# Vasilispapg/CVML-GoalNet

Measured on AMD Instinct MI355X. Metric: training clips/sec at batch 64, 16-frame 224² clips; logit MAE vs CPU ref, higher is better.
Workload: dtype f32; 1 GPU; AVM train step (forward + broadcast-MSE + backward + fused Adam), 64 clips x 16 frames = 1024 frames of 3x224x224 + 30x30 MFCC per GPU; dropout live (device masks), BatchNorm train mode; frames_per_gpu=1024, h=224, w=224, parallelism=dp1, ddp_semantics=local BN + local MSE per rank, gradient mean (standard DDP), params=1286754369

## Files before the change

cvml_goalnet_amd/_lib.py:

```python
from __future__ import annotations

import ctypes
import os
from ctypes import c_char_p, c_double, c_float, c_int, c_int64, c_size_t, c_uint32, c_uint64, c_void_p

_HERE = os.path.dirname(os.path.abspath(__file__))
LIB_PATH = os.environ.get("GOALNET_LIB_PATH") or os.path.join(_HERE, "libgoalnet_hip.so")
ABI_VERSION = 7
STAT_PARTS = 1024
ADAM_RANGES_MAX = 32

P = c_void_p


class RowCopy(ctypes.Structure):
    _fields_ = [("src", c_void_p), ("dst", c_void_p), ("row_bytes", c_int64), ("nrows", c_int), ("gather", c_int), ("cursor", c_void_p),
                ("cursor_bias", c_int64)]


class AdamRange(ctypes.Structure):
    _fields_ = [("begin", c_int64), ("count", c_int64), ("skipped", c_int64)]


PROTOTYPES = {
# ... 63 lines not shown
    "goalnet_linear_bwd_dx_split": (c_int, [c_int, P, P, P, c_int64, c_int, c_int64, c_int, P, P]),
    "goalnet_linear_bwd_dw_split": (c_int, [c_int, P, P, P, c_int, c_int64, c_int, P, P]),
    "goalnet_linear_bwd_dx_bf16": (c_int, [P, c_int64, P, P, c_int64, P, c_int64, c_int, c_int64, c_int, c_int, P]),
    "goalnet_linear_bwd_dx_bf16_o16_ok": (c_int, [c_int, c_int64, c_int]),
    "goalnet_linear_bwd_dx_bf16_o16": (c_int, [P, c_int64, P, P, c_int64, c_int, c_int64, c_int, c_int, P]),
    "goalnet_conv3x3_fwd_bf16p_o16_ok": (c_int, [c_int, c_int, c_int, c_int, c_int]),
    "goalnet_conv3x3_fwd_bf16p_o16": (c_int, [P, P, P, c_int, P, c_int, c_int, c_int, c_int, c_int, c_int, P]),
    "goalnet_linear_bwd_dw_bf16": (c_int, [P, c_int64, P, c_int64, P, c_int, c_int64, c_int, c_int, P]),
    "goalnet_linear_fwd_ws_bytes": (c_size_t, [c_int, c_int64, c_int]),
    "goalnet_linear_fwd": (c_int, [P, c_int64, P, P, c_int, P, P, c_int, P, c_int64, P, c_int64, P, c_int64,
                                   c_int, c_int64, c_int, P, c_size_t, P]),
    "goalnet_linear_bwd_dx": (c_int, [P, c_int64, P, P, c_int64, P, c_int64, c_int, c_int64, c_int, P]),
    "goalnet_linear_bwd_dw": (c_int, [P, c_int64, P, c_int64, P, P, c_int, P, P, c_int, c_int64, c_int, P]),
    "goalnet_linear_bwd_dw_adam": (c_int, [P, c_int64, P, c_int64, P, P, c_int, P, P, P, P, c_int, c_int64, c_int,
                                           c_double, c_double, c_double, c_double, P, c_int64, c_float, P]),
    "goalnet_colsum": (c_int, [P, c_int64, c_int, c_int, P, P]),
    "goalnet_mul": (c_int, [P, c_int64, P, c_int64, P, c_int64, c_int, c_int, P]),
    "goalnet_conv1d_fwd": (c_int, [P, P, P, c_int, P, c_int, c_int, c_int, c_int, c_int, c_int, P]),
    "goalnet_conv1d_bwd_ws_bytes": (c_size_t, [c_int, c_int, c_int]),
    "goalnet_conv1d_bwd": (c_int, [P, P, P, P, P, P, c_int, c_int, c_int, c_int, c_int, c_int, P, c_size_t, P]),
    "goalnet_conv1d_bwd_small": (c_int, [P, P, P, P, P, P, P, c_int, c_int, c_int, c_int, c_int, c_int, P]),
    "goalnet_relu_bwd": (c_int, [P, P, P, c_int64, P]),
    "goalnet_mlp_blocks": (c_int, []),
    "goalnet_mlp_fwd": (c_int, [P, c_int64, c_int, P, P, P, P, P, P, P, P, P, P, P, c_int, P, P]),
    "goalnet_mlp_bwd_ws_bytes": (c_size_t, [c_int]),
    "goalnet_mlp_bwd": (c_int, [P, P, P, c_int64, P, c_int64, P, P, P, P, c_int64, P, c_int, c_int, c_int, P, c_size_t, P, P]),
    "goalnet_head_fwd": (c_int, [P, c_int64, P, P, P, P, c_int, c_int, P]),
    "goalnet_head_bwd": (c_int, [P, P, P, c_int64, P, P, c_int64, P, c_int64, P, P, c_int, c_int, P]),
    "goalnet_mse_bcast": (c_int, [P, P, c_int, P, P, P]),
    "goalnet_cubic_resample": (c_int, [P, P, P, c_int64, c_int, c_int, P]),
# ... 75 lines not shown
```

cvml_goalnet_amd/avm.py:

```python
from __future__ import annotations

import math
import os
from typing import List, Optional

import torch
import torch.nn as nn
from torch.nn.parameter import UninitializedParameter

from . import ops
from ._lib import GoalnetError
from .synth import BASE_SEED, DROP_P, TID_DROP

F32 = torch.float32
BN_EPS = 1e-5
BN_MOMENTUM = 0.1
_ALIGN = 64


class _LazyFlags:

    def requires_grad_(self, requires_grad: bool = True):
        for p in self.parameters():
            p.requires_grad = requires_grad
# ... 56 lines not shown
            torch.cuda.current_stream().wait_event(ev)

    def join(self):
        if self.enabled and self.forked:
            torch.cuda.current_stream().wait_stream(self.side)
            self.forked = False
        self.keep.clear()


class _Bwd:

    def __init__(self, model, train, fork):
        self.model, self.train, self.fork = model, train, fork
        self.scratch = {}
        self.dbias = {}
        self.T = train.__contains__

    def any_T(self, *layers):
        return any(f"{layer}.{leaf}" in self.train for layer in layers for leaf in ("weight", "bias"))

    def G(self, name):
        m = self.model
        if name in self.train:
            return m._gflat(name)
        s = m.spec(name)
        if s.kind in ("ohwi", "lin5") and name != "visbl.conv1.weight":
            raise GoalnetError(f"a backward that does not train {name} asked for its gradient")
        t = self.scratch.get(name)
        if t is None:
            t = self.scratch[name] = torch.empty(s.numel, dtype=F32, device=m._device)
# ... 34 lines not shown
    if env == "0":
        return frozenset()
    return frozenset(ch for ch in env.lower() if ch in "a")


def epi_fuse_dw_adam(n, *, plain, synced, precision, train_w5, shadowed, inspected, forced, pieces):
    if forced is False or "a" not in pieces:
        return False
    if inspected and forced is not True:
        return False
    if not (plain and not synced and precision == "fp32" and train_w5 and not shadowed):
        return False
    if n <= EPI_FUSE_SKINNY_ROWS:
        return False
    return forced is True or n >= EPI_FUSE_MIN_ROWS


class AVM(_LazyFlags, nn.Module):
    def __init__(self, audio_included, device=None, seed: Optional[int] = None, precision: str = "fp32", head: str = "regression",
                 num_classes: int = 5):
        super().__init__()
        self.audio_included = audio_included
        if head not in ("regression", "classifier"):
            raise ValueError("head must be 'regression' (the reference's live code) or 'classifier' (its commented-out variant)")
        if not 2 <= num_classes <= 8:
            raise ValueError("num_classes must be in 2..8")
        self.head = head
        self.num_classes = num_classes if head == "classifier" else 1
        if precision not in ("fp32", "bf16", "fp16", "bf16x6", "fp16x3"):
            raise ValueError("precision must be 'fp32' (the reference's arithmetic), 'bf16x6' / 'fp16x3' (fp32 operands as bf16 triples / scaled "
# ... 44 lines not shown
        self.grad_sync = None
        self.stat_sync = None
        self.grad_bf16 = os.environ.get("GOALNET_DZ16", "1") != "0"
        self.act_bf16 = os.environ.get("GOALNET_P16", "1") != "0"
        env = os.environ.get
        self.x6_off = env("GOALNET_X6_OFF") == "1"
        self.x6_linear5 = env("GOALNET_X6_LINEAR5", "1") != "0"
        self.x3_wgrad2 = env("GOALNET_X3_WGRAD2", "1") != "0"
        self.x3_dgrad2 = env("GOALNET_X3_DGRAD2", "1") != "0"
        self.mlp_fused = env("GOALNET_MLP_FUSED", "1") != "0"
        self.small_bn = env("GOALNET_SMALL_BN", "1") != "0"
        self.force_bf5 = env("GOALNET_FORCE_BF5") == "1"
        self.overlap_pair = env("GOALNET_OVERLAP_PAIR", "1") != "0"
        self.epi_fuse = None
        self.epi_fused_dw = 0
        self.keep_ctx = False
        self.last_ctx = None
        self.last_used_w5b = False
        self._side_stream = None
        self.overlap_rows = int(os.environ.get("GOALNET_OVERLAP_ROWS", "64"))
        _ol = os.environ.get("GOALNET_OVERLAP_LARGE")
        self.overlap_large = _ol == "1"
        self.overlap_auto = _ol is None
        self.time_labels = None
        self.kernel_events = None

    @property
    def precision(self) -> str:
        return self._precision

# ... 350 lines not shown
        return self._x6 and ops.linear_split_ok(self._parts, n, k5, 512) and not self.x6_off and self.x6_linear5

    def _mlp_fused(self, n):
        return n <= 16 and self.head == "regression" and self.mlp_fused

    def _bf5(self, n):
        return self._half and (n > 16 or self.force_bf5)

    def _pair(self, n):
        return self._large_overlap(n) and self.overlap_pair

    def _small_bn(self, a, b, n, hc, wc, c):
        return (a.dtype == F32 and b.dtype == F32 and self.stat_sync is None and c <= 512 and n * hc * wc * c <= ops.SMALL_BN_ELEMS
                and self.small_bn)

    def _bn_block(self, y, n, hc, wc, c, i, save, p16=False):
        dev = self._device
        assert p16 or y.dtype == F32
        p = torch.empty(n, hc - 2, wc - 2, c, dtype=self._h16 if p16 else F32, device=dev)
        idx = torch.empty(n, hc - 2, wc - 2, c, dtype=torch.uint8, device=dev) if save else None
        bn = getattr(self.visbl, f"bnorm{i}")
        st = torch.empty(4, c, dtype=F32, device=dev)
        count = n * (hc - 2) * (wc - 2)
        if not self.training:
            ops.pool_bn_eval_fwd(y, p, idx, self._pflat(f"visbl.bnorm{i}.weight"), self._pflat(f"visbl.bnorm{i}.bias"),
                                 bn.running_mean, bn.running_var, BN_EPS, st, n, hc, wc, c)
            return p, idx, st
        if self._small_bn(y, p, n, hc, wc, c):
            ops.pool_bn_fwd_small(y, p, idx, self._pflat(f"visbl.bnorm{i}.weight"), self._pflat(f"visbl.bnorm{i}.bias"),
                                  bn.running_mean, bn.running_var, BN_MOMENTUM, BN_EPS, st, n, hc, wc, c)
# ... 145 lines not shown
        elif not fused_mlp:
            logit = torch.empty(n, dtype=F32, device=dev)
            out = torch.empty(n, dtype=F32, device=dev)
            ops.head_fwd(x, P("fusion.12.weight"), P("fusion.12.bias"), logit, out)
        if save:
            ctx.update(p1=p1, idx1=idx1, st1=st1, p2=p2, idx2=idx2, st2=st2, p3=p3, idx3=idx3, st3=st3,
                       a1=a1, a2=a2, hs=hs, ms=ms, logit=logit, out=out, l1=l1, l2=l2)
        self.last_logit = logit
        self.last_features = cat
        return out, ctx

    def _block_bwd(self, bwd, dbn, ctx, i, n, hc, wc, c):
        dev, G, bias = self._device, bwd.G, bwd.T(f"visbl.conv{i}.bias")
        p, idx, st = ctx[f"p{i}"], ctx[f"idx{i}"], ctx[f"st{i}"]
        npix = n * (hc - 2) * (wc - 2)
        small = self._small_bn(dbn, p, n, hc, wc, c) and not (self._half and i > 1)
        frozen = ctx["eval"]
        if small:
            coef3 = torch.empty(3 * c, dtype=F32, device=dev)
            (ops.bn_bwd_reduce_small_eval if frozen else ops.bn_bwd_reduce_small)(
                dbn, p, st[0], st[1], self._pflat(f"visbl.bnorm{i}.weight"), G(f"visbl.bnorm{i}.weight"), G(f"visbl.bnorm{i}.bias"),
                coef3, n, hc, wc, c)
            dy = torch.empty(n, hc, wc, c, dtype=F32, device=dev)
            dparts = torch.empty(ops.stat_parts(8 * n) * c, dtype=torch.float64, device=dev)
            ops.bnpool_bwd(dbn, p, idx, coef3, dy, dparts, n, hc, wc, c)
            if i > 1 and bias:
                bwd.dbias[i] = (dparts, c)
            return dy
        coef3 = torch.empty(3 * c, dtype=F32, device=dev)
        partials = torch.empty(ops.stat_parts(npix // 64) * 2 * c, dtype=torch.float64, device=dev)
        ops.bn_bwd_reduce(dbn, p, st[0], st[1], partials, npix, c)
        if frozen:
            ops.bn_bwd_finalize_eval(partials, self._pflat(f"visbl.bnorm{i}.weight"), st[1], c,
                                     G(f"visbl.bnorm{i}.weight"), G(f"visbl.bnorm{i}.bias"), coef3)
        else:
            ops.bn_bwd_finalize(partials, self._pflat(f"visbl.bnorm{i}.weight"), st[0], st[1], npix, c,
                                G(f"visbl.bnorm{i}.weight"), G(f"visbl.bnorm{i}.bias"), coef3)
        if self.stat_sync is not None and not frozen:
            scratch = torch.empty(2 * c, dtype=F32, device=dev)
            ops.bn_bwd_finalize(self._global_sums(partials, 2 * c), self._pflat(f"visbl.bnorm{i}.weight"), st[0], st[1],
                                npix * self.stat_sync.world, c, scratch[:c], scratch[c:], coef3)
        dparts = torch.empty(ops.stat_parts(8 * n) * c, dtype=torch.float64, device=dev)
        if self._half and i > 1 and self._bwd16_ok(wc):
            dy = self._padbuf(f"dy{i}", n, hc, wc, c)
            ops.bnpool_bwd_bf16p(dbn, p, idx, coef3, None, dy, dparts, n, hc, wc, c)
        elif self._half and i > 1:
# ... 45 lines not shown
            return None
        if flipped:
            fork.wait(wait_ev)
        else:
            ops.conv3x3_weight_flip(P(wname), wt, cout, cin)
        o16 = out16 and ops.conv3x3_fwd_bf16p_o16_ok(n, hc, wc, cout, cin)
        dx = torch.empty(n, hc, wc, cin, dtype=self._h16 if o16 else F32, device=dev)
        if self._half:
            wtb = ops.cast_bf16(wt, torch.empty(wt.shape, dtype=self._h16, device=dev))
            self._timed("conv_dgrad", flops, ops.conv3x3_fwd_bf16p_o16 if o16 else ops.conv3x3_fwd_bf16p,
                        dy, wtb, None, False, dx, n, hc, wc, cout, cin)
        elif split and split_dgrad:
            wts, awt = self._split_w(wt, cin * 9, cout)
            self._timed("conv_dgrad", flops, ops.conv3x3_fwd_split, self._parts,
                        dys, wts, None, False, dx, n, hc, wc, cout, cin, self._osc(ady, awt))
        else:
            self._timed("conv_dgrad", flops, ops.conv3x3_fwd, dy, None, None, wt, None, False, dx, n, hc, wc, cout, cin)
        if pair:
            wgrad()
        return dx

    def backward_device(self, ctx, dout, on_bucket=None, after_linear5=None, inputs=None, params=True, reduce=0, frozen=None,
                        fused_w5=None):
        need_aud, need_vis = inputs if inputs is not None else (False, False)
        need_aud = need_aud and self.audio_included
        train = frozenset()
        if params:
            frozen = self._frozen_names() if frozen is None else frozenset(frozen)
            self._check_freeze(frozen)
            train = frozenset(s.name for s in self._specs) - frozen
# ... 2 lines not shown
                               "backward ran; call backward after each forward (as the reference's loop does)")
        for i in (3, 2):
            xs = f"x{i - 1}s"
            if not self._half and xs in ctx and f"visbl.conv{i}.weight" in train and ctx[xs + "_gen"] != self._padgen[xs]:
                raise RuntimeError(f"precision='{self.precision}': a second training-mode forward overwrote the saved split operands "
                                   "before backward ran; call backward after each forward (as the reference's loop does)")
        if params:
            self._ensure_garena()
            self._bwd_frozen = frozen
        dev = self._device
        n, h, w = ctx["n"], ctx["h"], ctx["w"]
        bwd = _Bwd(self, train, _Fork(self, self._fork_ok(n) and dout.is_cuda))
        fork, T, G, any_T = bwd.fork, bwd.T, bwd.G, bwd.any_T
        (h1, w1), (hp1, wp1), (hp2, wp2), (hp3, wp3) = self._sizes(h, w)
        P = self._pflat
        need_b1 = need_vis or any_T("visbl.bnorm1", "visbl.conv1")
        need_b2 = need_b1 or any_T("visbl.bnorm2", "visbl.conv2")
        need_b3 = need_b2 or any_T("visbl.bnorm3", "visbl.conv3")
        train_w5 = T("visbl.linear5.weight")
        need_audbl = self.audio_included and (need_aud or any_T("audbl.linear3", "audbl.conv2", "audbl.conv1"))
        need_cat = need_audbl or need_b3 or train_w5 or T("visbl.linear5.bias")
        d_audio = torch.empty(n, 30, ctx["bins"], dtype=F32, device=dev) if need_aud else None
        d_visual = None
        hs, ms = ctx["hs"], ctx["ms"]
        pair = fork.enabled and self._pair(n)
        deferred_l5 = []

        def bucket_done(k):
            if on_bucket:
                fork.join()
# ... 89 lines not shown
                else:
                    ops.linear_bwd_dx_bf16(dz5b, ctx["w5b"], dbn3.view(n, k5), mult=None)
            elif "x3s" in ctx:
                dz5s, adz = self._split_mat(dz5, n, 512)
                if train_w5:
                    osc_w = self._osc(adz, ctx["x3s_amax"])
                    fork.run(lambda: ops.linear_bwd_dw_split(self._parts, dz5s, ctx["x3s"], G("visbl.linear5.weight"), n, k5, 512, oscale=osc_w), dz5s, osc_w)
                bucket_done(1)
                if need_b3:
                    ops.linear_bwd_dx_split(self._parts, dz5s, ctx["w5s"], dbn3.view(n, k5), n, k5, 512, oscale=self._osc(adz, ctx["w5s_amax"]))
            else:
                fuse5 = fused_w5 is not None and train_w5
                if train_w5 and not fuse5:
                    fork.run(lambda: ops.linear_bwd_dw(dz5, p3f, G("visbl.linear5.weight"), scale=st3[2], shift=st3[3], bnC=512), dz)
                bucket_done(1)
                if need_b3:
                    ops.linear_bwd_dx(dz5, P("visbl.linear5.weight"), dbn3.view(n, k5), mult=None)
                if fuse5:
                    fused_w5(dz5, p3f, st3[2], st3[3])
            linear5_done()
        else:
            bucket_done(1)

        b2, b3 = (hp1, wp1, 64, 256), (hp2, wp2, 256, 512)
        dbn2 = dbn1 = None
        if dbn3 is not None:
            dbn2 = self._conv_block_bwd(bwd, 3, dbn3, ctx, n, *b3, wt3, flips_early, flips_ev, pair, out16=dz16 and self._bwd16_ok(wp1),
                                        split_dgrad=True, after_block=lambda: [cb(fork) for cb in deferred_l5], dgrad=need_b2)
        del dbn3
        if dbn2 is not None:
            dbn1 = self._conv_block_bwd(bwd, 2, dbn2, ctx, n, *b2, wt2, flips_early, None, pair, out16=False,
# ... 323 lines not shown
```

cvml_goalnet_amd/csrc/gemm_f32.hip:

```cpp
#include <stdlib.h>

#include "adam.h"
#include "gemm_common.h"
#include "skinny.h"

using namespace goalnet;

namespace {

constexpr int BM = 128, BN = 128, BK = 32;
constexpr int LDR = 128;
constexpr int OP_FLOATS = BM * BK;

__device__ __forceinline__ int kc_off(int row, int chunk) { return row * BK + ((chunk ^ ((row >> 1) & 7)) << 2); }

__device__ __forceinline__ float4 f4zero() { return make_float4(0.f, 0.f, 0.f, 0.f); }
__device__ __forceinline__ float4 f4fma(float4 v, float4 s, float4 t) {
    return make_float4(fmaf(v.x, s.x, t.x), fmaf(v.y, s.y, t.y), fmaf(v.z, s.z, t.z), fmaf(v.w, s.w, t.w));
}

typedef unsigned int u32x4 __attribute__((ext_vector_type(4)));
constexpr unsigned OOB = 0xFFFFFF00u;

__device__ __forceinline__ float4 f4sel(bool v, float4 a) { return v ? a : f4zero(); }
// ... 716 lines not shown
                adam1(pp[q].x, acc[fm][0][e], mm[q].x, vv[q].x, s.b2, s.omb1, s.omb2, ae.eps, s.step_size, s.bc2_sqrt, ae.gs);
                adam1(pp[q].y, acc[fm][1][e], mm[q].y, vv[q].y, s.b2, s.omb1, s.omb2, ae.eps, s.step_size, s.bc2_sqrt, ae.gs);
            }
#pragma unroll
            for (int q = 0; q < 4; ++q) {
                if (ok[q]) {
                    *reinterpret_cast<float2*>(ae.p + idx[q]) = pp[q];
                    *reinterpret_cast<float2*>(ae.m + idx[q]) = mm[q];
                    *reinterpret_cast<float2*>(ae.v + idx[q]) = vv[q];
                }
            }
        }
    }
}

template <class AL, class BL, int STAGES, int EPI>
__global__ __launch_bounds__(256, STAGES == 1 ? AL::ONE_STAGE_BLOCKS : 2) void gemm_f32_epi_kernel(typename AL::P ap, typename BL::P bp, AdamEpi ae,
                                                          int rows, int cols, int64_t ld, int tiles_m, int tiles_n, int m_fast, int ktiles) {
    static_assert(EPI == EPIK_ADAM && !AL::KC && !BL::KC, "the Adam epilogue: both operands row-contiguous");
    const int tid = threadIdx.x;
    int tm, tn;
    tile_of_block(tiles_m, tiles_n, m_fast, tm, tn);
    AdamScalars s = adam_scalars(ae.lr, ae.beta1, ae.beta2, *ae.step + ae.step_bias);
    s.step_size = wave_uniform(s.step_size); s.bc2_sqrt = wave_uniform(s.bc2_sqrt);
    s.b2 = wave_uniform(s.b2); s.omb1 = wave_uniform(s.omb1); s.omb2 = wave_uniform(s.omb2);
    const int lane = tid & 63, wave = tid >> 6;
    const int wm = wave >> 1, wn = wave & 1;
    const int r = lane & 31, h = lane >> 5;
    f32x16 acc[2][2];
    gemm_mainloop<AL, BL, STAGES>(ap, bp, tm, tn, 0, ktiles, tid, acc);
    adam_acc(ae, s, rows, cols, ld, acc, tm, tn, wm, wn, r, h);
}

template <class AL, class BL, int EPI>
int launch_gemm_epi(const char* name, const typename AL::P& ap, const typename BL::P& bp, const AdamEpi& ae, int64_t M, int64_t N,
                    int64_t ld, int ktiles, int m_fast, hipStream_t st) {
    const int64_t tiles_m = (M + BM - 1) / BM, tiles_n = (N + BN - 1) / BN;
    GN_REQUIRE(tiles_m * tiles_n < (1ll << 31), GOALNET_E_SHAPE, "%s: too many tiles", name);
    static const int force_stages = getenv("GOALNET_F32_STAGES") ? atoi(getenv("GOALNET_F32_STAGES")) : 0;
    const dim3 grid((unsigned)(tiles_m * tiles_n), 1, 1);
    if (force_stages == 1 || (force_stages != 2 && AL::ONE_STAGE))
        hipLaunchKernelGGL((gemm_f32_epi_kernel<AL, BL, 1, EPI>), grid, dim3(256), 0, st, ap, bp, ae, (int)M, (int)N, ld, (int)tiles_m,
                           (int)tiles_n, m_fast, ktiles);
    else
        hipLaunchKernelGGL((gemm_f32_epi_kernel<AL, BL, 2, EPI>), grid, dim3(256), 0, st, ap, bp, ae, (int)M, (int)N, ld, (int)tiles_m,
                           (int)tiles_n, m_fast, ktiles);
    GN_LAUNCH_CHECK(name);
    return 0;
}

__global__ __launch_bounds__(256) void splitk_reduce_kernel(const float* slabs, int nsplit, int64_t slab_stride, EpiP ep) {
    const int c4n = ep.cols >> 2;
    const int64_t total = (int64_t)ep.rows * c4n;
    for (int64_t i = (int64_t)blockIdx.x * blockDim.x + threadIdx.x; i < total; i += (int64_t)gridDim.x * blockDim.x) {
        const int64_t row = i / c4n;
        const int col = (int)(i - row * c4n) * 4;
        const float* s = slabs + row * ep.cols + col;
        float4 a = *reinterpret_cast<const float4*>(s);
        for (int k = 1; k < nsplit; ++k) {
            const float4 b = *reinterpret_cast<const float4*>(s + (int64_t)k * slab_stride);
            a.x += b.x; a.y += b.y; a.z += b.z; a.w += b.w;
// ... 416 lines not shown
               GOALNET_E_ALIGN, "linear_bwd_dw_adam: pointers / leading dims must be 16-byte aligned");
    GN_REQUIRE(aligned16(p) && aligned16(m) && aligned16(v), GOALNET_E_ALIGN, "linear_bwd_dw_adam: p, m and v must be 16-byte aligned");
    hipStream_t st = (hipStream_t)stream;
    if (db) { const int rc = goalnet_colsum(dy, lddy, M, J, db, stream); if (rc) return rc; }
    const int ktiles = (M + BK - 1) / BK;
    MCLoader<false>::P ap{dy, lddy, J, M, nullptr, nullptr, 1};
    const AdamEpi ae{p, m, v, lr, beta1, beta2, (float)eps, grad_scale, step, step_bias};
    if (scale) {
        MCLoader<true>::P bp{x, ldx, (int)K, M, scale, shift, bnC};
        return launch_gemm_epi<MCLoader<false>, MCLoader<true>, EPIK_ADAM>("linear_bwd_dw_adam", ap, bp, ae, J, K, K, ktiles, 1, st);
    }
    MCLoader<false>::P bp{x, ldx, (int)K, M, nullptr, nullptr, 1};
    return launch_gemm_epi<MCLoader<false>, MCLoader<false>, EPIK_ADAM>("linear_bwd_dw_adam", ap, bp, ae, J, K, K, ktiles, 1, st);
}

}
```

cvml_goalnet_amd/csrc/pool_bn.hip:

```cpp
#include <hip/hip_bf16.h>
#include <stdlib.h>

#include "common.h"

using namespace goalnet;

namespace {

constexpr int PARTS = GOALNET_STAT_PARTS;

struct d4 { double x, y, z, w; };

template <int NV>
__device__ __forceinline__ void block_reduce_store(double (&v)[NV][4], int G, int tid, double* smem,
                                                   double* out_row, int64_t out_stride, int C) {
#pragma unroll
    for (int a = 0; a < NV; ++a)
#pragma unroll
        for (int c = 0; c < 4; ++c) smem[tid * (NV * 4) + a * 4 + c] = v[a][c];
    __syncthreads();
    if (tid < G) {
        const int reps = 256 / G;
#pragma unroll
        for (int a = 0; a < NV; ++a)
// ... 868 lines not shown
    const int c = blockIdx.x * 16 + (threadIdx.x & 15);
    const double s = column_sum16(partials + c, nparts, stride, c < C, sm);
    if (c < C && threadIdx.x < 16) out[c] = (float)s;
}

__global__ __launch_bounds__(256) void partials_sum2_kernel(const double* __restrict__ pa, int na, int Ca, float* __restrict__ oa, int blocks_a,
                                                           const double* __restrict__ pb, int nb, int Cb, float* __restrict__ ob) {
    __shared__ double sm[256];
    const bool first = (int)blockIdx.x < blocks_a;
    const double* partials = first ? pa : pb;
    const int nparts = first ? na : nb, C = first ? Ca : Cb;
    float* out = first ? oa : ob;
    const int c = (first ? blockIdx.x : blockIdx.x - blocks_a) * 16 + (threadIdx.x & 15);
    const double s = column_sum16(partials + c, nparts, C, c < C, sm);
    if (c < C && threadIdx.x < 16) out[c] = (float)s;
}

__global__ __launch_bounds__(256) void partials_sum_f64_kernel(const double* __restrict__ partials, int nparts, int64_t stride,
                                                              int C, double* __restrict__ out) {
    __shared__ double sm[256];
    const int c = blockIdx.x * 16 + (threadIdx.x & 15);
    const double s = column_sum16(partials + c, nparts, stride, c < C, sm);
    if (c < C && threadIdx.x < 16) out[c] = s;
}

int row_bands(int nparts, int N, int rows) {
    int b = nparts / N;
    if (b > rows / 3) b = rows / 3;
    return b < 1 ? 1 : b;
}
// ... 354 lines not shown
    GN_REQUIRE(nparts > 0 && C > 0 && stride >= C, GOALNET_E_SHAPE, "partials_sum: bad dims");
    hipLaunchKernelGGL(partials_sum_kernel, dim3((C + 15) / 16), dim3(256), 0, (hipStream_t)stream, partials, nparts, stride, C, out);
    GN_LAUNCH_CHECK("partials_sum");
    return 0;
}

int goalnet_partials_sum2(const double* pa, int na, int Ca, float* oa, const double* pb, int nb, int Cb, float* ob, void* stream) {
    GN_REQUIRE(pa && oa && pb && ob, GOALNET_E_NULL, "partials_sum2: null pointer");
    GN_REQUIRE(na > 0 && Ca > 0 && nb > 0 && Cb > 0, GOALNET_E_SHAPE, "partials_sum2: bad dims");
    const int ba = (Ca + 15) / 16, bb = (Cb + 15) / 16;
    hipLaunchKernelGGL(partials_sum2_kernel, dim3(ba + bb), dim3(256), 0, (hipStream_t)stream, pa, na, Ca, oa, ba, pb, nb, Cb, ob);
    GN_LAUNCH_CHECK("partials_sum2");
    return 0;
}

int goalnet_partials_sum_f64(const double* partials, int nparts, int64_t stride, int C, double* out, void* stream) {
    GN_REQUIRE(partials && out, GOALNET_E_NULL, "partials_sum_f64: null pointer");
    GN_REQUIRE(nparts > 0 && C > 0 && stride >= C, GOALNET_E_SHAPE, "partials_sum_f64: bad dims");
    hipLaunchKernelGGL(partials_sum_f64_kernel, dim3((C + 15) / 16), dim3(256), 0, (hipStream_t)stream, partials, nparts, stride, C, out);
    GN_LAUNCH_CHECK("partials_sum_f64");
    return 0;
}

}
```

cvml_goalnet_amd/ops.py:

```python
from __future__ import annotations

import ctypes
import os

import torch

from . import _lib
from ._lib import STAT_PARTS, check

F32 = torch.float32


def _s():
    return torch.cuda.current_stream().cuda_stream


def _p(t):
    return 0 if t is None else t.data_ptr()


def _chk(*ts):
    for t in ts:
        if t is None:
            continue
# ... 582 lines not shown
    check(lib().goalnet_linear_bwd_dw(dy.data_ptr(), _ld(dy), x.data_ptr(), _ld(x), _p(scale), _p(shift), bnC, dw.data_ptr(), _p(db),
                                      M, K, J, _s()), "linear_bwd_dw")
    return dw


def linear_bwd_dw_adam(dy, x, p, m, v, lr, beta1, beta2, eps, step, *, scale=None, shift=None, bnC=0, db=None, grad_scale=1.0, step_bias=0):
    _chk(dy, x, p, m, v, scale, shift, db)
    M, J = dy.shape
    K = x.shape[1]
    _req(p.numel() == J * K and m.numel() == J * K and v.numel() == J * K and x.shape[0] == M and (db is None or db.numel() == J),
         "linear_bwd_dw_adam: argument check failed: p.numel() == m.numel() == v.numel() == J * K and x.shape[0] == M and (db is None or db.numel() == J)")
    _req(p.is_contiguous() and m.is_contiguous() and v.is_contiguous(), "linear_bwd_dw_adam: p, m and v must be contiguous")
    check(lib().goalnet_linear_bwd_dw_adam(dy.data_ptr(), _ld(dy), x.data_ptr(), _ld(x), _p(scale), _p(shift), bnC, p.data_ptr(), m.data_ptr(),
                                           v.data_ptr(), _p(db), M, K, J, lr, beta1, beta2, eps, _ctr(step), int(step_bias), grad_scale, _s()),
          "linear_bwd_dw_adam")


def colsum(x, out):
    _chk(x, out)
    M, J = x.shape
    _req(out.numel() == J, "colsum: argument check failed: out.numel() == J")
    check(lib().goalnet_colsum(x.data_ptr(), _ld(x), M, J, out.data_ptr(), _s()), "colsum")
    return out


def mul(x, m, y):
    _chk(x, m, y)
    M, J = x.shape
    check(lib().goalnet_mul(x.data_ptr(), _ld(x), m.data_ptr(), _ld(m), y.data_ptr(), _ld(y), M, J, _s()), "mul")
    return y
# ... 325 lines not shown
```

include/goalnet_hip.h:

```cpp
#ifndef GOALNET_HIP_H
#define GOALNET_HIP_H

#include <stddef.h>
#include <stdint.h>

#ifdef __cplusplus
extern "C" {
#endif

#define GOALNET_ABI_VERSION 7

#define GOALNET_OK 0
#define GOALNET_E_NULL (-1)
#define GOALNET_E_SHAPE (-2)
#define GOALNET_E_ALIGN (-3)
#define GOALNET_E_WORKSPACE (-4)

#define GOALNET_STAT_PARTS 1024
int goalnet_stat_parts(int64_t units);

int goalnet_abi_version(void);
const char* goalnet_last_error(void);

int goalnet_fill_uniform(float* dst, int64_t n, uint64_t seed, uint32_t tensor_id, float lo, float hi, void* stream);
// ... 119 lines not shown
size_t goalnet_linear_fwd_ws_bytes(int M, int64_t K, int J);
int goalnet_linear_fwd(const float* x, int64_t ldx, const float* scale, const float* shift, int bnC,
                       const float* w, const float* bias, int relu, const float* dropmask, int64_t ldmask,
                       float* y, int64_t ldy, float* mult_out, int64_t ldmult,
                       int M, int64_t K, int J, void* ws, size_t ws_bytes, void* stream);
int goalnet_linear_bwd_dx(const float* dy, int64_t lddy, const float* w, const float* mult, int64_t ldmult,
                          float* dx, int64_t lddx, int M, int64_t K, int J, void* stream);
int goalnet_linear_bwd_dw(const float* dy, int64_t lddy, const float* x, int64_t ldx,
                          const float* scale, const float* shift, int bnC,
                          float* dw, float* db, int M, int64_t K, int J, void* stream);
int goalnet_linear_bwd_dw_adam(const float* dy, int64_t lddy, const float* x, int64_t ldx,
                               const float* scale, const float* shift, int bnC,
                               float* p, float* m, float* v, float* db, int M, int64_t K, int J,
                               double lr, double beta1, double beta2, double eps, const int64_t* step, int64_t step_bias,
                               float grad_scale, void* stream);
int goalnet_colsum(const float* x, int64_t ldx, int M, int J, float* out, void* stream);
int goalnet_mul(const float* x, int64_t ldx, const float* mult, int64_t ldmult, float* y, int64_t ldy,
                int M, int J, void* stream);

int goalnet_conv1d_fwd(const float* x, const float* w, const float* b, int relu, float* y,
                       int N, int Cin, int L, int Cout, int stride, int pad, void* stream);
size_t goalnet_conv1d_bwd_ws_bytes(int N, int Cin, int Cout);
int goalnet_conv1d_bwd(const float* x, const float* dz, const float* w, float* dx, float* dw, float* db,
                       int N, int Cin, int L, int Cout, int stride, int pad, void* ws, size_t ws_bytes, void* stream);
int goalnet_conv1d_bwd_small(const float* x, const float* dz, const float* y, const float* w, float* dx, float* dw, float* db,
                             int N, int Cin, int L, int Cout, int stride, int pad, void* stream);
int goalnet_relu_bwd(const float* dy, const float* y, float* dz, int64_t n, void* stream);

int goalnet_mlp_blocks(void);
int goalnet_mlp_fwd(const float* cat, int64_t ldcat, int K0, const float* const* w, const float* const* b,
// ... 111 lines not shown
```

Baseline: 159.8 clips/s.

## Fuse BatchNorm backward sums into linear5 dx and conv3 dgrad epilogues

Adds a GEMM epilogue that, while storing the dgrad/dx output, also accumulates per-tile fp64 sums of dy and dy·x̂ for the upstream BatchNorm. A small fold kernel then turns these tile partials into the stat partials, so the separate bn_bwd_reduce pass over the large activation and gradient tensors is skipped for blocks 3 and 2. This is meant to save a full re-read of dbn and p. In exchange the epilogue adds register pressure and extra global reads of p inside the GEMM, and allocates a new tileparts buffer.

```diff
diff --git a/cvml_goalnet_amd/_lib.py b/cvml_goalnet_amd/_lib.py
--- a/cvml_goalnet_amd/_lib.py
+++ b/cvml_goalnet_amd/_lib.py
@@ -101,6 +101,11 @@
     "goalnet_linear_bwd_dw": (c_int, [P, c_int64, P, c_int64, P, P, c_int, P, P, c_int, c_int64, c_int, P]),
     "goalnet_linear_bwd_dw_adam": (c_int, [P, c_int64, P, c_int64, P, P, c_int, P, P, P, P, c_int, c_int64, c_int,
                                            c_double, c_double, c_double, c_double, P, c_int64, c_float, P]),
+    "goalnet_bn_tileparts_bytes_dx": (c_size_t, [c_int, c_int64, c_int]),
+    "goalnet_bn_tileparts_bytes_conv": (c_size_t, [c_int, c_int, c_int, c_int, c_int]),
+    "goalnet_linear_bwd_dx_bnsums": (c_int, [P, c_int64, P, P, c_int64, P, c_int64, P, P, c_int, P, c_size_t, c_int, c_int64, c_int, P]),
+    "goalnet_conv3x3_dgrad_bnsums": (c_int, [P, P, P, P, P, P, P, c_size_t, c_int, c_int, c_int, c_int, c_int, P]),
+    "goalnet_bn_tileparts_fold": (c_int, [P, c_int, c_int64, c_int, P, c_int, P]),
     "goalnet_colsum": (c_int, [P, c_int64, c_int, c_int, P, P]),
     "goalnet_mul": (c_int, [P, c_int64, P, c_int64, P, c_int64, c_int, c_int, P]),
     "goalnet_conv1d_fwd": (c_int, [P, P, P, c_int, P, c_int, c_int, c_int, c_int, c_int, c_int, P]),
diff --git a/cvml_goalnet_amd/avm.py b/cvml_goalnet_amd/avm.py
--- a/cvml_goalnet_amd/avm.py
+++ b/cvml_goalnet_amd/avm.py
@@ -94,6 +94,8 @@
         self.model, self.train, self.fork = model, train, fork
         self.scratch = {}
         self.dbias = {}
+        self.bnsums = frozenset()
+        self.tileparts = {}
         self.T = train.__contains__
 
     def any_T(self, *layers):
@@ -158,6 +160,27 @@
     if n <= EPI_FUSE_SKINNY_ROWS:
         return False
     return forced is True or n >= EPI_FUSE_MIN_ROWS
+
+
+def epi_bnsums_pieces(env):
+    if env is None or env in ("", "1"):
+        return frozenset("bc")
+    if env == "0":
+        return frozenset()
+    return frozenset(ch for ch in env.lower() if ch in "bc")
+
+
+def epi_bnsums_blocks(n, *, fp32, synced, small3, small2, served3, served2, unsplit2, forced, pieces):
+    if forced is False or not fp32 or synced:
+        return frozenset()
+    if forced is not True and n < EPI_FUSE_MIN_ROWS:
+        return frozenset()
+    blocks = set()
+    if "b" in pieces and served3 and not small3:
+        blocks.add(3)
+    if "c" in pieces and served2 and not small2 and (unsplit2 or forced is True):
+        blocks.add(2)
+    return frozenset(blocks)
 
 
 class AVM(_LazyFlags, nn.Module):
@@ -232,6 +255,8 @@
         self.overlap_pair = env("GOALNET_OVERLAP_PAIR", "1") != "0"
         self.epi_fuse = None
         self.epi_fused_dw = 0
+        self.epi_bnsums = None
+        self.epi_bnsums_used = {3: 0, 2: 0}
         self.keep_ctx = False
         self.last_ctx = None
         self.last_used_w5b = False
@@ -612,6 +637,20 @@
         return (a.dtype == F32 and b.dtype == F32 and self.stat_sync is None and c <= 512 and n * hc * wc * c <= ops.SMALL_BN_ELEMS
                 and self.small_bn)
 
+    def _epi_bnsums(self, ctx, n, hp1, wp1, hp2, wp2):
+        p3, p2 = ctx.get("p3"), ctx.get("p2")
+        if self.epi_bnsums is False or p3 is None or p2 is None:
+            return frozenset()
+        fp32 = self.precision == "fp32" and not self._half and p3.dtype == F32 and p2.dtype == F32 and "x3s" not in ctx and "x2s" not in ctx
+        lib = ops.lib()
+        return epi_bnsums_blocks(
+            n, fp32=fp32, synced=self.stat_sync is not None,
+            small3=self._small_bn(p3, p3, n, hp2, wp2, 512), small2=self._small_bn(p2, p2, n, hp1, wp1, 256),
+            served3=ops.bn_tileparts_bytes_dx(n, 512 * (hp2 - 2) * (wp2 - 2), 512) > 0,
+            served2=ops.bn_tileparts_bytes_conv(n, hp2, wp2, 512, 256) > 0,
+            unsplit2=lib.goalnet_conv3x3_fwd_ws_bytes(n, hp2, wp2, 512, 256) == 0,
+            forced=self.epi_bnsums, pieces=epi_bnsums_pieces(os.environ.get("GOALNET_F32_EPI_BNSUMS")))
+
     def _bn_block(self, y, n, hc, wc, c, i, save, p16=False):
         dev = self._device
         assert p16 or y.dtype == F32
@@ -787,7 +826,8 @@
         dev, G, bias = self._device, bwd.G, bwd.T(f"visbl.conv{i}.bias")
         p, idx, st = ctx[f"p{i}"], ctx[f"idx{i}"], ctx[f"st{i}"]
         npix = n * (hc - 2) * (wc - 2)
-        small = self._small_bn(dbn, p, n, hc, wc, c) and not (self._half and i > 1)
+        tiles = bwd.tileparts.pop(i, None)
+        small = tiles is None and self._small_bn(dbn, p, n, hc, wc, c) and not (self._half and i > 1)
         frozen = ctx["eval"]
         if small:
             coef3 = torch.empty(3 * c, dtype=F32, device=dev)
@@ -802,7 +842,12 @@
             return dy
         coef3 = torch.empty(3 * c, dtype=F32, device=dev)
         partials = torch.empty(ops.stat_parts(npix // 64) * 2 * c, dtype=torch.float64, device=dev)
-        ops.bn_bwd_reduce(dbn, p, st[0], st[1], partials, npix, c)
+        if tiles is not None:
+            ops.bn_tileparts_fold(tiles[0], tiles[1], tiles[2], c, partials)
+            self.epi_bnsums_used[i] += 1
+        else:
+            ops.bn_bwd_reduce(dbn, p, st[0], st[1], partials, npix, c)
+        del tiles
         if frozen:
             ops.bn_bwd_finalize_eval(partials, self._pflat(f"visbl.bnorm{i}.weight"), st[1], c,
                                      G(f"visbl.bnorm{i}.weight"), G(f"visbl.bnorm{i}.bias"), coef3)
@@ -878,6 +923,11 @@
             wts, awt = self._split_w(wt, cin * 9, cout)
             self._timed("conv_dgrad", flops, ops.conv3x3_fwd_split, self._parts,
                         dys, wts, None, False, dx, n, hc, wc, cout, cin, self._osc(ady, awt))
+        elif i - 1 in bwd.bnsums:
+            st_in = ctx[f"st{i - 1}"]
+            tp = torch.empty(ops.bn_tileparts_bytes_conv(n, hc, wc, cout, cin) // 8, dtype=torch.float64, device=dev)
+            self._timed("conv_dgrad", flops, ops.conv3x3_dgrad_bnsums, dy, wt, dx, ctx[f"p{i - 1}"], st_in[0], st_in[1], tp, n, hc, wc, cout, cin)
+            bwd.tileparts[i - 1] = (tp, (n * hc * wc + 127) // 128, cin)
         else:
             self._timed("conv_dgrad", flops, ops.conv3x3_fwd, dy, None, None, wt, None, False, dx, n, hc, wc, cout, cin)
         if pair:
@@ -910,6 +960,7 @@
         fork, T, G, any_T = bwd.fork, bwd.T, bwd.G, bwd.any_T
         (h1, w1), (hp1, wp1), (hp2, wp2), (hp3, wp3) = self._sizes(h, w)
         P = self._pflat
+        bwd.bnsums = self._epi_bnsums(ctx, n, hp1, wp1, hp2, wp2)
         need_b1 = need_vis or any_T("visbl.bnorm1", "visbl.conv1")
         need_b2 = need_b1 or any_T("visbl.bnorm2", "visbl.conv2")
         need_b3 = need_b2 or any_T("visbl.bnorm3", "visbl.conv3")
@@ -1029,7 +1080,12 @@
                 if train_w5 and not fuse5:
                     fork.run(lambda: ops.linear_bwd_dw(dz5, p3f, G("visbl.linear5.weight"), scale=st3[2], shift=st3[3], bnC=512), dz)
                 bucket_done(1)
-                if need_b3:
+                if need_b3 and 3 in bwd.bnsums:
+                    tp3 = torch.empty(ops.bn_tileparts_bytes_dx(n, k5, 512) // 8, dtype=torch.float64, device=dev)
+                    ops.linear_bwd_dx_bnsums(dz5, P("visbl.linear5.weight"), dbn3.view(n, k5), p3f, st3[0], st3[1], 512, tp3)
+                    bwd.tileparts[3] = (tp3, (n + 127) // 128, k5)
+                    del tp3
+                elif need_b3:
                     ops.linear_bwd_dx(dz5, P("visbl.linear5.weight"), dbn3.view(n, k5), mult=None)
                 if fuse5:
                     fused_w5(dz5, p3f, st3[2], st3[3])
diff --git a/cvml_goalnet_amd/csrc/gemm_f32.hip b/cvml_goalnet_amd/csrc/gemm_f32.hip
--- a/cvml_goalnet_amd/csrc/gemm_f32.hip
+++ b/cvml_goalnet_amd/csrc/gemm_f32.hip
@@ -754,37 +754,154 @@
     }
 }
 
+enum { EPIK_BNSUMS = 2 };
+
+struct BnSumsEpi {
+    float* out;
+    const float* p; int64_t ldp;
+    const float* mean; const float* invstd; int C;
+    double* tileparts;
+};
+
+template <int EPI> struct EpiArgs { using T = AdamEpi; };
+template <> struct EpiArgs<EPIK_BNSUMS> { using T = BnSumsEpi; };
+
+template <bool BIL>
+__device__ __forceinline__ void bnsums_acc(const BnSumsEpi& be, int rows, int cols, int64_t ld, const f32x16 (&acc)[2][2],
+                                           int tm, int tn, int wm, int wn, int r, int h, double* red) {
+    int col[2];
+    bool colok[2];
+    float mu[2], is[2];
+    double s[2] = {0.0, 0.0}, q[2] = {0.0, 0.0};
+#pragma unroll
+    for (int fn = 0; fn < 2; ++fn) {
+        col[fn] = tn * GEMM_BN + wn * 64 + (BIL ? 2 * r + fn : fn * 32 + r);
+        colok[fn] = col[fn] < cols;
+        const int c = (colok[fn] ? col[fn] : 0) % be.C;
+        mu[fn] = be.mean[c];
+        is[fn] = be.invstd[c];
+    }
+#pragma unroll
+    for (int fm = 0; fm < 2; ++fm) {
+        const int row0 = tm * GEMM_BM + wm * 64 + fm * 32 + 4 * h;
+#pragma unroll
+        for (int eb = 0; eb < 2; ++eb) {
+            float x[8][2];
+#pragma unroll
+            for (int i = 0; i < 8; ++i) {
+                const int e = 8 * eb + i;
+                const int row = row0 + (e & 3) + 8 * (e >> 2);
+                if (BIL) {
+                    const float2 t = *reinterpret_cast<const float2*>(be.p + (colok[0] && row < rows ? (int64_t)row * be.ldp + col[0] : 0));
+                    x[i][0] = t.x; x[i][1] = t.y;
+                } else {
+#pragma unroll
+                    for (int fn = 0; fn < 2; ++fn) x[i][fn] = be.p[colok[fn] && row < rows ? (int64_t)row * be.ldp + col[fn] : 0];
+                }
+            }
+#pragma unroll
+            for (int i = 0; i < 8; ++i) {
+                const int e = 8 * eb + i;
+                const int row = row0 + (e & 3) + 8 * (e >> 2);
+                const bool rowok = row < rows;
+                if (BIL) {
+                    if (colok[0] && rowok) *reinterpret_cast<float2*>(be.out + (int64_t)row * ld + col[0]) = make_float2(acc[fm][0][e], acc[fm][1][e]);
+                } else {
+#pragma unroll
+                    for (int fn = 0; fn < 2; ++fn)
+                        if (colok[fn] && rowok) be.out[(int64_t)row * ld + col[fn]] = acc[fm][fn][e];
+                }
+#pragma unroll
+                for (int fn = 0; fn < 2; ++fn) {
+                    const bool ok = colok[fn] && rowok;
+                    const double d = (double)acc[fm][fn][e];
+                    const float xh = (x[i][fn] - mu[fn]) * is[fn];
+                    s[fn] += ok ? d : 0.0;
+                    q[fn] += ok ? d * (double)xh : 0.0;
+                }
+            }
+        }
+    }
+    const int slot = (wn * 64 + (BIL ? 2 * r : r)) * 2;
+    constexpr int FS = BIL ? 2 : 64;
+#pragma unroll
+    for (int fn = 0; fn < 2; ++fn) {
+        s[fn] += __shfl_xor(s[fn], 32);
+        q[fn] += __shfl_xor(q[fn], 32);
+        if (wm == 1 && h == 0) { red[slot + fn * FS] = s[fn]; red[slot + fn * FS + 1] = q[fn]; }
+    }
+    __syncthreads();
+    if (wm == 0 && h == 0) {
+#pragma unroll
+        for (int fn = 0; fn < 2; ++fn) {
+            if (!colok[fn]) continue;
+            double* tp = be.tileparts + (int64_t)tm * 2 * cols + col[fn];
+            tp[0] = s[fn] + red[slot + fn * FS];
+            tp[cols] = q[fn] + red[slot + fn * FS + 1];
+        }
+    }
+}
+
 template <class AL, class BL, int STAGES, int EPI>
-__global__ __launch_bounds__(256, STAGES == 1 ? AL::ONE_STAGE_BLOCKS : 2) void gemm_f32_epi_kernel(typename AL::P ap, typename BL::P bp, AdamEpi ae,
+__global__ __launch_bounds__(256, STAGES == 1 ? AL::ONE_STAGE_BLOCKS : 2) void gemm_f32_epi_kernel(typename AL::P ap, typename BL::P bp, typename EpiArgs<EPI>::T ae,
                                                           int rows, int cols, int64_t ld, int tiles_m, int tiles_n, int m_fast, int ktiles) {
-    static_assert(EPI == EPIK_ADAM && !AL::KC && !BL::KC, "the Adam epilogue: both operands row-contiguous");
+    static_assert(EPI == EPIK_ADAM || EPI == EPIK_BNSUMS, "unknown epilogue");
     const int tid = threadIdx.x;
     int tm, tn;
     tile_of_block(tiles_m, tiles_n, m_fast, tm, tn);
-    AdamScalars s = adam_scalars(ae.lr, ae.beta1, ae.beta2, *ae.step + ae.step_bias);
-    s.step_size = wave_uniform(s.step_size); s.bc2_sqrt = wave_uniform(s.bc2_sqrt);
-    s.b2 = wave_uniform(s.b2); s.omb1 = wave_uniform(s.omb1); s.omb2 = wave_uniform(s.omb2);
-    const int lane = tid & 63, wave = tid >> 6;
-    const int wm = wave >> 1, wn = wave & 1;
-    const int r = lane & 31, h = lane >> 5;
-    f32x16 acc[2][2];
-    gemm_mainloop<AL, BL, STAGES>(ap, bp, tm, tn, 0, ktiles, tid, acc);
-    adam_acc(ae, s, rows, cols, ld, acc, tm, tn, wm, wn, r, h);
+    if constexpr (EPI == EPIK_ADAM) {
+        static_assert(EPI != EPIK_ADAM || (!AL::KC && !BL::KC), "the Adam epilogue: both operands row-contiguous");
+        AdamScalars s = adam_scalars(ae.lr, ae.beta1, ae.beta2, *ae.step + ae.step_bias);
+        s.step_size = wave_uniform(s.step_size); s.bc2_sqrt = wave_uniform(s.bc2_sqrt);
+        s.b2 = wave_uniform(s.b2); s.omb1 = wave_uniform(s.omb1); s.omb2 = wave_uniform(s.omb2);
+        const int lane = tid & 63, wave = tid >> 6;
+        const int wm = wave >> 1, wn = wave & 1;
+        const int r = lane & 31, h = lane >> 5;
+        f32x16 acc[2][2];
+        gemm_mainloop<AL, BL, STAGES>(ap, bp, tm, tn, 0, ktiles, tid, acc);
+        adam_acc(ae, s, rows, cols, ld, acc, tm, tn, wm, wn, r, h);
+    } else {
+        static_assert(EPI != EPIK_BNSUMS || AL::KC, "the BatchNorm-sums epilogue: rows in store_acc's plain order");
+        const int lane = tid & 63, wave = tid >> 6;
+        const int wm = wave >> 1, wn = wave & 1;
+        const int r = lane & 31, h = lane >> 5;
+        f32x16 acc[2][2];
+        if constexpr (AL::STRIP) {
+            static_assert(STAGES == 1 && BL::KC, "the strip form: one B stage");
+            AL al(ap, tm * BM, tid);
+            BL bl(bp, tn * BN, tid);
+#pragma unroll
+            for (int i = 0; i < 2; ++i)
+#pragma unroll
+                for (int j = 0; j < 2; ++j)
+#pragma unroll
+                    for (int e = 0; e < 16; ++e) acc[i][j][e] = 0.f;
+            __shared__ __attribute__((aligned(16))) float lstrip[STRIP_FLOATS];
+            __shared__ __attribute__((aligned(16))) float lbs[OP_FLOATS];
+            conv_strip_loop(al, bl, lstrip, lbs, acc, ktiles, tid, wn, r, h);
+            bnsums_acc<false>(ae, rows, cols, ld, acc, tm, tn, wm, wn, r, h, reinterpret_cast<double*>(lbs));
+        } else {
+            __shared__ double red[256];
+            gemm_mainloop<AL, BL, STAGES>(ap, bp, tm, tn, 0, ktiles, tid, acc);
+            bnsums_acc<!BL::KC>(ae, rows, cols, ld, acc, tm, tn, wm, wn, r, h, red);
+        }
+    }
 }
 
 template <class AL, class BL, int EPI>
-int launch_gemm_epi(const char* name, const typename AL::P& ap, const typename BL::P& bp, const AdamEpi& ae, int64_t M, int64_t N,
+int launch_gemm_epi(const char* name, const typename AL::P& ap, const typename BL::P& bp, const typename EpiArgs<EPI>::T& ae, int64_t M, int64_t N,
                     int64_t ld, int ktiles, int m_fast, hipStream_t st) {
     const int64_t tiles_m = (M + BM - 1) / BM, tiles_n = (N + BN - 1) / BN;
     GN_REQUIRE(tiles_m * tiles_n < (1ll << 31), GOALNET_E_SHAPE, "%s: too many tiles", name);
     static const int force_stages = getenv("GOALNET_F32_STAGES") ? atoi(getenv("GOALNET_F32_STAGES")) : 0;
     const dim3 grid((unsigned)(tiles_m * tiles_n), 1, 1);
-    if (force_stages == 1 || (force_stages != 2 && AL::ONE_STAGE))
+    if (AL::STRIP || force_stages == 1 || (force_stages != 2 && AL::ONE_STAGE)) {
         hipLaunchKernelGGL((gemm_f32_epi_kernel<AL, BL, 1, EPI>), grid, dim3(256), 0, st, ap, bp, ae, (int)M, (int)N, ld, (int)tiles_m,
                            (int)tiles_n, m_fast, ktiles);
-    else
+    } else if constexpr (!AL::STRIP) {
         hipLaunchKernelGGL((gemm_f32_epi_kernel<AL, BL, 2, EPI>), grid, dim3(256), 0, st, ap, bp, ae, (int)M, (int)N, ld, (int)tiles_m,
                            (int)tiles_n, m_fast, ktiles);
+    }
     GN_LAUNCH_CHECK(name);
     return 0;
 }
@@ -1231,4 +1348,58 @@
     return launch_gemm_epi<MCLoader<false>, MCLoader<false>, EPIK_ADAM>("linear_bwd_dw_adam", ap, bp, ae, J, K, K, ktiles, 1, st);
 }
 
-}
+size_t goalnet_bn_tileparts_bytes_dx(int M, int64_t K, int C) {
+    if (M <= SKINNY_MAX_M || K <= 0 || K >= (1ll << 31) - 256 || C <= 0 || C % 4 != 0 || K % C != 0) return 0;
+    return (size_t)((M + BM - 1) / BM) * 2 * (size_t)K * sizeof(double);
+}
+
+size_t goalnet_bn_tileparts_bytes_conv(int N, int H, int W, int Cin, int Cout) {
+    if (N <= 0 || H <= 0 || W <= 0 || Cin <= 0 || Cout <= 0 || Cin % BK != 0 || Cout % 4 != 0) return 0;
+    const int64_t M = (int64_t)N * H * W;
+    if (M >= (1ll << 31) - 256) return 0;
+    const bool narrow = Cout <= 64 && !getenv("GOALNET_F32_N64_OFF");
+    if (!conv_strip_f32(W, 1, narrow, false)) return 0;
+    return (size_t)((M + BM - 1) / BM) * 2 * (size_t)Cout * sizeof(double);
+}
+
+int goalnet_linear_bwd_dx_bnsums(const float* dy, int64_t lddy, const float* w, float* dx, int64_t lddx,
+                                 const float* p, int64_t ldp, const float* mean, const float* invstd, int C,
+                                 double* tileparts, size_t tileparts_bytes, int M, int64_t K, int J, void* stream) {
+    GN_REQUIRE(dy && w && dx && p && mean && invstd && tileparts, GOALNET_E_NULL, "linear_bwd_dx_bnsums: null pointer");
+    GN_REQUIRE(M > 0 && J > 0 && K > 0 && K < (1ll << 31) - 256, GOALNET_E_SHAPE, "linear_bwd_dx_bnsums: bad dims");
+    GN_REQUIRE(J % BK == 0, GOALNET_E_SHAPE, "linear_bwd_dx_bnsums: J=%d must be a multiple of %d", J, BK);
+    GN_REQUIRE(K % 4 == 0, GOALNET_E_SHAPE, "linear_bwd_dx_bnsums: K must be a multiple of 4");
+    GN_REQUIRE(C > 0 && C % 4 == 0 && K % C == 0, GOALNET_E_SHAPE, "linear_bwd_dx_bnsums: C=%d must be a multiple of 4 that divides K", C);
+    GN_REQUIRE(M > SKINNY_MAX_M, GOALNET_E_SHAPE, "linear_bwd_dx_bnsums: M=%d is served by the weight-streaming kernels (M > %d here)", M, SKINNY_MAX_M);
+    GN_REQUIRE(aligned16(dy) && aligned16(w) && aligned16(dx) && aligned16(p) && aligned16(mean) && aligned16(invstd) &&
+               lddy % 4 == 0 && lddx % 4 == 0 && ldp % 4 == 0, GOALNET_E_ALIGN, "linear_bwd_dx_bnsums: pointers / leading dims must be 16-byte aligned");
+    GN_REQUIRE((reinterpret_cast<uintptr_t>(tileparts) & 7u) == 0, GOALNET_E_ALIGN, "linear_bwd_dx_bnsums: tileparts must be 8-byte aligned");
+    GN_REQUIRE(tileparts_bytes >= goalnet_bn_tileparts_bytes_dx(M, K, C), GOALNET_E_WORKSPACE, "linear_bwd_dx_bnsums: tileparts too small");
+    KCLoader<false>::P ap{dy, lddy, M, nullptr, nullptr, 1, 0};
+    MCLoader<false>::P bp{w, K, (int)K, J, nullptr, nullptr, 1};
+    const BnSumsEpi be{dx, p, ldp, mean, invstd, C, tileparts};
+    return launch_gemm_epi<KCLoader<false>, MCLoader<false>, EPIK_BNSUMS>("linear_bwd_dx_bnsums", ap, bp, be, M, K, lddx, J / BK, 1, (hipStream_t)stream);
+}
+
+int goalnet_conv3x3_dgrad_bnsums(const float* dy, const float* wflipped, float* dx, const float* p, const float* mean, const float* invstd,
+                                 double* tileparts, size_t tileparts_bytes, int N, int H, int W, int Cin, int Cout, void* stream) {
+    GN_REQUIRE(dy && wflipped && dx && p && mean && invstd && tileparts, GOALNET_E_NULL, "conv3x3_dgrad_bnsums: null pointer");
+    GN_REQUIRE(N > 0 && H > 0 && W > 0 && Cin > 0 && Cout > 0, GOALNET_E_SHAPE, "conv3x3_dgrad_bnsums: non-positive dim");
+    GN_REQUIRE(Cin % BK == 0, GOALNET_E_SHAPE, "conv3x3_dgrad_bnsums: Cin=%d must be a multiple of %d", Cin, BK);
+    GN_REQUIRE(Cout % 4 == 0, GOALNET_E_SHAPE, "conv3x3_dgrad_bnsums: Cout=%d must be a multiple of 4", Cout);
+    const int64_t M = (int64_t)N * H * W;
+    GN_REQUIRE(M < (1ll << 31) - 256, GOALNET_E_SHAPE, "conv3x3_dgrad_bnsums: N*H*W too large");
+    const size_t need = goalnet_bn_tileparts_bytes_conv(N, H, W, Cin, Cout);
+    GN_REQUIRE(need > 0, GOALNET_E_SHAPE, "conv3x3_dgrad_bnsums: served by the strip form of the 128 x 128 tile only (Cout > 64, W <= %d)", CONV_STRIP_MAX_W);
+    GN_REQUIRE(aligned16(dy) && aligned16(wflipped) && aligned16(dx) && aligned16(p) && aligned16(mean) && aligned16(invstd),
+               GOALNET_E_ALIGN, "conv3x3_dgrad_bnsums: pointers must be 16-byte aligned");
+    GN_REQUIRE((reinterpret_cast<uintptr_t>(tileparts) & 7u) == 0, GOALNET_E_ALIGN, "conv3x3_dgrad_bnsums: tileparts must be 8-byte aligned");
+    GN_REQUIRE(tileparts_bytes >= need, GOALNET_E_WORKSPACE, "conv3x3_dgrad_bnsums: tileparts too small");
+    ConvAStripLoader<false>::P ap{dy, H, W, Cin, M, nullptr, nullptr};
+    KCLoader<false>::P bp{wflipped, (int64_t)9 * Cin, Cout, nullptr, nullptr, 1, Cin};
+    const BnSumsEpi be{dx, p, Cout, mean, invstd, Cout, tileparts};
+    return launch_gemm_epi<ConvAStripLoader<false>, KCLoader<false>, EPIK_BNSUMS>("conv3x3_dgrad_bnsums", ap, bp, be, M, Cout, Cout, 9 * Cin / BK, 0,
+                                                                                  (hipStream_t)stream);
+}
+
+}
diff --git a/cvml_goalnet_amd/csrc/pool_bn.hip b/cvml_goalnet_amd/csrc/pool_bn.hip
--- a/cvml_goalnet_amd/csrc/pool_bn.hip
+++ b/cvml_goalnet_amd/csrc/pool_bn.hip
@@ -906,6 +906,27 @@
     const int c = (first ? blockIdx.x : blockIdx.x - blocks_a) * 16 + (threadIdx.x & 15);
     const double s = column_sum16(partials + c, nparts, C, c < C, sm);
     if (c < C && threadIdx.x < 16) out[c] = (float)s;
+}
+
+__global__ __launch_bounds__(256) void bn_tileparts_fold_kernel(const double* __restrict__ tileparts, int tile_rows, int64_t cols, int C,
+                                                               double* __restrict__ partials, int nparts) {
+    const int wc = blockIdx.y * 256 + threadIdx.x;
+    if (wc >= 2 * C) return;
+    const int which = wc >= C ? 1 : 0, c = wc - which * C;
+    const int64_t npx = cols / C, entries = (int64_t)tile_rows * npx;
+    const int j = blockIdx.x;
+    const auto at = [&](int64_t e) {
+        const int64_t tr = e / npx, px = e - tr * npx;
+        return tileparts[(tr * 2 + which) * cols + px * C + c];
+    };
+    double acc = 0.0;
+    int64_t e = j;
+    for (; e + 3 * (int64_t)nparts < entries; e += 4 * (int64_t)nparts) {
+        const double a0 = at(e), a1 = at(e + nparts), a2 = at(e + 2 * (int64_t)nparts), a3 = at(e + 3 * (int64_t)nparts);
+        acc += a0; acc += a1; acc += a2; acc += a3;
+    }
+    for (; e < entries; e += nparts) acc += at(e);
+    partials[(int64_t)j * 2 * C + wc] = acc;
 }
 
 __global__ __launch_bounds__(256) void partials_sum_f64_kernel(const double* __restrict__ partials, int nparts, int64_t stride,
@@ -1290,6 +1311,18 @@
     return 0;
 }
 
+int goalnet_bn_tileparts_fold(const double* tileparts, int tile_rows, int64_t cols, int C, double* partials, int nparts, void* stream) {
+    GN_REQUIRE(tileparts && partials, GOALNET_E_NULL, "bn_tileparts_fold: null pointer");
+    GN_REQUIRE(tile_rows > 0 && C > 0 && cols > 0 && cols % C == 0, GOALNET_E_SHAPE, "bn_tileparts_fold: cols must be a positive multiple of C");
+    GN_PARTS_OK("bn_tileparts_fold");
+    GN_REQUIRE((reinterpret_cast<uintptr_t>(tileparts) & 7u) == 0 && (reinterpret_cast<uintptr_t>(partials) & 7u) == 0, GOALNET_E_ALIGN,
+               "bn_tileparts_fold: pointers must be 8-byte aligned");
+    hipLaunchKernelGGL(bn_tileparts_fold_kernel, dim3(nparts, (2 * C + 255) / 256), dim3(256), 0, (hipStream_t)stream, tileparts, tile_rows,
+                       cols, C, partials, nparts);
+    GN_LAUNCH_CHECK("bn_tileparts_fold");
+    return 0;
+}
+
 int goalnet_partials_sum_f64(const double* partials, int nparts, int64_t stride, int C, double* out, void* stream) {
     GN_REQUIRE(partials && out, GOALNET_E_NULL, "partials_sum_f64: null pointer");
     GN_REQUIRE(nparts > 0 && C > 0 && stride >= C, GOALNET_E_SHAPE, "partials_sum_f64: bad dims");
diff --git a/cvml_goalnet_amd/ops.py b/cvml_goalnet_amd/ops.py
--- a/cvml_goalnet_amd/ops.py
+++ b/cvml_goalnet_amd/ops.py
@@ -620,6 +620,47 @@
     check(lib().goalnet_linear_bwd_dw_adam(dy.data_ptr(), _ld(dy), x.data_ptr(), _ld(x), _p(scale), _p(shift), bnC, p.data_ptr(), m.data_ptr(),
                                            v.data_ptr(), _p(db), M, K, J, lr, beta1, beta2, eps, _ctr(step), int(step_bias), grad_scale, _s()),
           "linear_bwd_dw_adam")
+
+
+def bn_tileparts_bytes_dx(M, K, C):
+    return lib().goalnet_bn_tileparts_bytes_dx(M, K, C)
+
+
+def bn_tileparts_bytes_conv(N, H, W, Cin, Cout):
+    return lib().goalnet_bn_tileparts_bytes_conv(N, H, W, Cin, Cout)
+
+
+def linear_bwd_dx_bnsums(dy, w, dx, p, mean, invstd, C, tileparts):
+    _chk(dy, w, dx, p, mean, invstd, tileparts)
+    M, J = dy.shape
+    K = dx.shape[1]
+    _req(w.numel() == J * K and dx.shape[0] == M and tuple(p.shape) == (M, K), "linear_bwd_dx_bnsums: w (J, K), dx and p (M, K)")
+    _req(dx.dtype == F32 and p.dtype == F32 and mean.numel() == C and invstd.numel() == C, "linear_bwd_dx_bnsums: fp32 dx / p, mean and invstd (C)")
+    _req(tileparts.dtype == torch.float64 and tileparts.is_contiguous(), "linear_bwd_dx_bnsums: tileparts must be contiguous fp64")
+    check(lib().goalnet_linear_bwd_dx_bnsums(dy.data_ptr(), _ld(dy), w.data_ptr(), dx.data_ptr(), _ld(dx), p.data_ptr(), _ld(p), mean.data_ptr(),
+                                             invstd.data_ptr(), C, tileparts.data_ptr(), tileparts.numel() * 8, M, K, J, _s()), "linear_bwd_dx_bnsums")
+    return dx
+
+
+def conv3x3_dgrad_bnsums(dy, wflipped, dx, p, mean, invstd, tileparts, N, H, W, Cin, Cout):
+    _chk(dy, wflipped, dx, p, mean, invstd, tileparts)
+    _req(dy.numel() == N * H * W * Cin and dx.numel() == p.numel() == N * H * W * Cout and wflipped.numel() == Cout * 9 * Cin,
+         "conv3x3_dgrad_bnsums: dy (N,H,W,Cin), dx and p (N,H,W,Cout), wflipped (Cout,9,Cin)")
+    _req(dx.dtype == F32 and p.dtype == F32 and dy.dtype == F32 and mean.numel() == Cout and invstd.numel() == Cout,
+         "conv3x3_dgrad_bnsums: fp32 tensors, mean and invstd (Cout)")
+    _req(tileparts.dtype == torch.float64 and tileparts.is_contiguous(), "conv3x3_dgrad_bnsums: tileparts must be contiguous fp64")
+    check(lib().goalnet_conv3x3_dgrad_bnsums(dy.data_ptr(), wflipped.data_ptr(), dx.data_ptr(), p.data_ptr(), mean.data_ptr(), invstd.data_ptr(),
+                                             tileparts.data_ptr(), tileparts.numel() * 8, N, H, W, Cin, Cout, _s()), "conv3x3_dgrad_bnsums")
+    return dx
+
+
+def bn_tileparts_fold(tileparts, tile_rows, cols, C, partials):
+    _chk(tileparts, partials)
+    _req(tileparts.dtype == torch.float64 and tileparts.is_contiguous() and tileparts.numel() >= tile_rows * 2 * cols,
+         "bn_tileparts_fold: tileparts holds tile_rows * 2 * cols doubles")
+    check(lib().goalnet_bn_tileparts_fold(tileparts.data_ptr(), tile_rows, cols, C, partials.data_ptr(), _rows(partials, 2 * C), _s()),
+          "bn_tileparts_fold")
+    return partials
 
 
 def colsum(x, out):
diff --git a/include/goalnet_hip.h b/include/goalnet_hip.h
--- a/include/goalnet_hip.h
+++ b/include/goalnet_hip.h
@@ -157,6 +157,14 @@
                                float* p, float* m, float* v, float* db, int M, int64_t K, int J,
                                double lr, double beta1, double beta2, double eps, const int64_t* step, int64_t step_bias,
                                float grad_scale, void* stream);
+size_t goalnet_bn_tileparts_bytes_dx(int M, int64_t K, int C);
+size_t goalnet_bn_tileparts_bytes_conv(int N, int H, int W, int Cin, int Cout);
+int goalnet_linear_bwd_dx_bnsums(const float* dy, int64_t lddy, const float* w, float* dx, int64_t lddx,
+                                 const float* p, int64_t ldp, const float* mean, const float* invstd, int C,
+                                 double* tileparts, size_t tileparts_bytes, int M, int64_t K, int J, void* stream);
+int goalnet_conv3x3_dgrad_bnsums(const float* dy, const float* wflipped, float* dx, const float* p, const float* mean, const float* invstd,
+                                 double* tileparts, size_t tileparts_bytes, int N, int H, int W, int Cin, int Cout, void* stream);
+int goalnet_bn_tileparts_fold(const double* tileparts, int tile_rows, int64_t cols, int C, double* partials, int nparts, void* stream);
 int goalnet_colsum(const float* x, int64_t ldx, int M, int J, float* out, void* stream);
 int goalnet_mul(const float* x, int64_t ldx, const float* mult, int64_t ldmult, float* y, int64_t ldy,
                 int M, int J, void* stream);
```

New measurement: 161.2 clips/s, median of 6. About the same (+0.9%).
